# EthanD11/RS-VIO

Hardware: AMD Instinct MI355X
Metric: stereo frames/sec (tracker+BA) on 752×480 EuRoC stream; BA ms/iter at window=10 (higher is better)
Workload: dtype f32 (tracker) / f64 (BA)

## Files before the change

rs-vio_amd/csrc/pyramid.hip:

```cpp
#include "pyramid.hpp"

namespace rsvio {

namespace {

constexpr int TW = 64;
constexpr int TH = 8;
constexpr int STRIP_COLS = 320;
constexpr size_t LDS_CAP = 64 << 10;

__device__ __forceinline__ float triangle_kernel(float x) {
    float ax = fabsf(x);
    return ax < 1.0f ? 1.0f - ax : 0.0f;
}

__global__ void make_taps_kernel(TapTable tab, int n_entries) {
    int e = blockIdx.x * blockDim.x + threadIdx.x;
    if (e >= n_entries) return;
    int in_len = tab.ent_in_len[e];
    int out_len = tab.ent_out_len[e];
    int o = tab.ent_out_idx[e];
    float ratio = (float)in_len / (float)out_len;
    float sratio = ratio < 1.0f ? 1.0f : ratio;
    float support = 1.0f * sratio;
    float inputc = ((float)o + 0.5f) * ratio;
    long long left = (long long)floorf(inputc - support);
    if (left < 0) left = 0;
    if (left > (long long)in_len - 1) left = in_len - 1;
    long long right = (long long)ceilf(inputc + support);
    if (right < left + 1) right = left + 1;
    if (right > (long long)in_len) right = in_len;
    inputc = inputc - 0.5f;
    int cnt = (int)(right - left);
    float* w = tab.weights + (size_t)e * tab.max_taps;
    float sum = 0.0f;
    for (int k = 0; k < cnt; ++k) {
        float wv = triangle_kernel(((float)(left + k) - inputc) / sratio);
        w[k] = wv;
        sum += wv;
    }
    for (int k = 0; k < cnt; ++k) w[k] = w[k] / sum;
    tab.left[e] = (int)left;
    tab.count[e] = cnt;
}

__global__ __launch_bounds__(256) void pyramid_kernel(PyrLaunch L, PyrIO io) {
    extern __shared__ uint32_t smem[];
    const int img = blockIdx.y;
    {
        const int fb = (int)blockIdx.x - (L.copy_blocks + L.tile_start[L.levels]);
        if (fb >= 0) {
            if (img == 0 && fb < io.fast_cells) {
                const uint8_t* s0 = io.psrc ? io.psrc : io.src[0];
                fast_cell(s0, io.fg, fb, nullptr, nullptr, 0, io.fast_pt, io.fast_aff,
                          reinterpret_cast<uint8_t*>(smem));
            }
            return;
        }
    }
    const uint8_t* __restrict__ src = io.psrc ? io.psrc + (size_t)img * L.w * L.h : io.src[img];
    uint8_t* __restrict__ dst_base = io.psrc ? io.pdst + (size_t)img * L.pyr_bytes : io.dst[img];
    int b = blockIdx.x;
    const bool aligned = ((reinterpret_cast<uintptr_t>(src) | reinterpret_cast<uintptr_t>(dst_base)) & 15) == 0;
    if (b < L.copy_blocks) {
        const size_t tot = (size_t)L.w * L.h;
        if (!aligned) {
            for (size_t i = (size_t)b * blockDim.x + threadIdx.x; i < tot; i += (size_t)L.copy_blocks * blockDim.x)
                dst_base[i] = src[i];
            return;
        }
        const size_t n16 = tot / 16;
        const uint4* s4 = reinterpret_cast<const uint4*>(src);
        uint4* d4 = reinterpret_cast<uint4*>(dst_base);
        for (size_t i = (size_t)b * blockDim.x + threadIdx.x; i < n16; i += (size_t)L.copy_blocks * blockDim.x)
            d4[i] = s4[i];
        size_t tail0 = n16 * 16;
        if (b == 0)
            for (size_t i = tail0 + threadIdx.x; i < tot; i += blockDim.x) dst_base[i] = src[i];
        return;
    }
    b -= L.copy_blocks;
    int lev = 1;
    while (lev < L.levels - 1 && b >= L.tile_start[lev + 1]) ++lev;
    b -= L.tile_start[lev];
    const int nw = (int)level_w(L.w, lev), nh = (int)level_h(L.h, lev);
    const int tw = L.tile_w[lev], th = L.tile_h[lev];
    const int tiles_x = (nw + tw - 1) / tw;
    const int tx = b % tiles_x, ty = b / tiles_x;
    const int ox0 = tx * tw, ox1 = min(ox0 + tw, nw);
    const int oy0 = ty * th, oy1 = min(oy0 + th, nh);
    const int rows = oy1 - oy0, cols_out = ox1 - ox0;
    const int hx = L.hx_ent[lev], vy = L.vy_ent[lev];
    const TapTable& T = L.tab;
    const int xl = T.left[hx + ox0];
    const int xr = T.left[hx + ox1 - 1] + T.count[hx + ox1 - 1];
    const int yl = T.left[vy + oy0];
    const int yr = T.left[vy + oy1 - 1] + T.count[vy + oy1 - 1];
    const int ncols = xr - xl, nrows = yr - yl;
    const int xa = xl & ~3, xoff = xl - xa;
    const int pd = (xr - xa + 3) >> 2;
    const bool direct = (L.direct >> lev) & 1;
    uint8_t* strip = reinterpret_cast<uint8_t*>(smem);
    if (!direct) {
        if (aligned && (L.w & 3) == 0) {
            const uint32_t* s32 = reinterpret_cast<const uint32_t*>(src);
            const int wd = (int)(L.w >> 2);
            for (int idx = threadIdx.x; idx < nrows * pd; idx += blockDim.x) {
                const int r = idx / pd, d = idx - r * pd;
                smem[idx] = s32[(size_t)(yl + r) * wd + (xa >> 2) + d];
            }
        } else {
            for (int idx = threadIdx.x; idx < nrows * pd * 4; idx += blockDim.x) {
                const int r = idx / (pd * 4), c = idx - r * pd * 4;
                strip[idx] = (xa + c < (int)L.w) ? src[(size_t)(yl + r) * L.w + xa + c] : 0;
            }
        }
    }
    float* tmp = reinterpret_cast<float*>(smem + (direct ? 0 : nrows * pd));
    __syncthreads();
    for (int idx = threadIdx.x; idx < rows * ncols; idx += blockDim.x) {
        const int r = idx / ncols, c = idx - r * ncols;
        const int e = vy + oy0 + r;
        const int vl = T.left[e], vc = T.count[e];
        const float* __restrict__ vw = T.weights + (size_t)e * T.max_taps;
        float acc = 0.0f;
        if (!direct) {
            const uint8_t* col = strip + (vl - yl) * pd * 4 + xoff + c;
            for (int k = 0; k < vc; ++k) acc += (float)col[k * pd * 4] * vw[k];
        } else {
            const uint8_t* __restrict__ col = src + (size_t)vl * L.w + xl + c;
            for (int k = 0; k < vc; k += 8) {
                float px[8];
#pragma unroll
                for (int u = 0; u < 8; ++u) px[u] = (k + u < vc) ? (float)col[(size_t)(k + u) * L.w] : 0.0f;
#pragma unroll
                for (int u = 0; u < 8; ++u)
                    if (k + u < vc) acc += px[u] * vw[k + u];
            }
        }
        tmp[r * ncols + c] = acc;
    }
    __syncthreads();
    uint8_t* __restrict__ dst = dst_base + level_offset(L.w, L.h, lev);
    for (int idx = threadIdx.x; idx < rows * cols_out; idx += blockDim.x) {
        const int r = idx / cols_out, c = idx - r * cols_out;
        const int e = hx + ox0 + c;
        const int hl = T.left[e] - xl, hc = T.count[e];
        const float* __restrict__ hw = T.weights + (size_t)e * T.max_taps;
        const float* __restrict__ row = tmp + r * ncols + hl;
        float acc = 0.0f;
        for (int k = 0; k < hc; ++k) acc += row[k] * hw[k];
        float cl = acc < 0.0f ? 0.0f : (acc > 255.0f ? 255.0f : acc);
        dst[(size_t)(oy0 + r) * nw + ox0 + c] = (uint8_t)roundf(cl);
    }
}

}

void PyramidPlan::init(int w_, int h_, int levels_) {
    w = w_;
    h = h_;
    levels = levels_;
    if (levels < 1 || levels > kMaxLevels) throw std::invalid_argument("levels must be in [1, 8]");
    if (w < 16 || h < 16) throw std::invalid_argument("image too small");
    std::vector<int> in_len, out_len, out_idx;
    float max_ratio = 1.0f;
    memset(&launch, 0, sizeof(launch));
    for (int i = 1; i < levels; ++i) {
        int nw = (int)level_w(w, i), nh = (int)level_h(h, i);
        if (nw < 1 || nh < 1) throw std::invalid_argument("too many levels for image size");
        launch.hx_ent[i] = (int)in_len.size();
        for (int o = 0; o < nw; ++o) { in_len.push_back(w); out_len.push_back(nw); out_idx.push_back(o); }
        launch.vy_ent[i] = (int)in_len.size();
        for (int o = 0; o < nh; ++o) { in_len.push_back(h); out_len.push_back(nh); out_idx.push_back(o); }
        float rx = (float)w / nw, ry = (float)h / nh;
        max_ratio = std::max(max_ratio, std::max(rx, ry));
        launch.tile_h[i] = std::max(1, std::min(TH, (int)(16.0f / ry)));
        launch.tile_w[i] = std::max(1, std::min(TW, (int)std::floor((STRIP_COLS - 2.0f * rx - 4.0f) / rx)));
    }
    n_entries = (int)in_len.size();
    max_taps = (int)std::ceil(2.0f * max_ratio) + 4;
    int tiles = 0;
    for (int i = 1; i < levels; ++i) {
        launch.tile_start[i] = tiles;
        int nw = (int)level_w(w, i), nh = (int)level_h(h, i);
        tiles += ((nw + launch.tile_w[i] - 1) / launch.tile_w[i]) * ((nh + launch.tile_h[i] - 1) / launch.tile_h[i]);
    }
    launch.tile_start[levels] = tiles;
    launch.copy_blocks = std::max(1, (int)(((size_t)w * h / 16 + 255) / 256 / 4));
    total_blocks = launch.copy_blocks + tiles;
    launch.w = (uint32_t)w;
    launch.h = (uint32_t)h;
    launch.levels = levels;
    launch.pyr_bytes = level_offset(w, h, levels);
    if (n_entries > 0) {
        i_in.alloc(n_entries); i_out.alloc(n_entries); i_idx.alloc(n_entries);
        d_left.alloc(n_entries); d_count.alloc(n_entries);
        d_w.alloc((size_t)n_entries * max_taps);
        RSVIO_HIP(hipMemcpy(i_in.p, in_len.data(), sizeof(int) * n_entries, hipMemcpyHostToDevice));
        RSVIO_HIP(hipMemcpy(i_out.p, out_len.data(), sizeof(int) * n_entries, hipMemcpyHostToDevice));
        RSVIO_HIP(hipMemcpy(i_idx.p, out_idx.data(), sizeof(int) * n_entries, hipMemcpyHostToDevice));
        TapTable t;
        t.left = d_left.p; t.count = d_count.p; t.weights = d_w.p; t.max_taps = max_taps;
        t.ent_in_len = i_in.p; t.ent_out_len = i_out.p; t.ent_out_idx = i_idx.p;
        hipLaunchKernelGGL(make_taps_kernel, dim3((n_entries + 255) / 256), dim3(256), 0, 0, t, n_entries);
        RSVIO_HIP(hipGetLastError());
        RSVIO_HIP(hipDeviceSynchronize());
        launch.tab = t;
        std::vector<int> left(n_entries), count(n_entries);
        RSVIO_HIP(hipMemcpy(left.data(), d_left.p, sizeof(int) * n_entries, hipMemcpyDeviceToHost));
        RSVIO_HIP(hipMemcpy(count.data(), d_count.p, sizeof(int) * n_entries, hipMemcpyDeviceToHost));
        for (int i = 1; i < levels; ++i) {
            const int nw = (int)level_w(w, i), nh = (int)level_h(h, i);
            const int tw = launch.tile_w[i], th = launch.tile_h[i];
            size_t strip = 0, vert = 0;
            for (int ox0 = 0; ox0 < nw; ox0 += tw) {
                const int ox1 = std::min(ox0 + tw, nw);
                const int xl = left[launch.hx_ent[i] + ox0];
                const int xr = left[launch.hx_ent[i] + ox1 - 1] + count[launch.hx_ent[i] + ox1 - 1];
                const size_t pd = (size_t)(xr - (xl & ~3) + 3) / 4;
                for (int oy0 = 0; oy0 < nh; oy0 += th) {
                    const int oy1 = std::min(oy0 + th, nh);
                    const int yl = left[launch.vy_ent[i] + oy0];
                    const int yr = left[launch.vy_ent[i] + oy1 - 1] + count[launch.vy_ent[i] + oy1 - 1];
                    strip = std::max(strip, 4 * pd * (size_t)(yr - yl));
                    vert = std::max(vert, 4 * (size_t)(oy1 - oy0) * (size_t)(xr - xl));
                }
            }
            if (vert > LDS_CAP) throw std::invalid_argument("image too wide for the pyramid tile");
            if (strip + vert > LDS_CAP) launch.direct |= 1u << i;
            lds_bytes = std::max(lds_bytes, ((launch.direct >> i) & 1) ? vert : strip + vert);
        }
    }
}

void PyramidPlan::enqueue(const PyrIO& io, int n_img, hipStream_t s) const {
    if (n_img <= 0) return;
    if (n_img > (io.psrc ? 65535 : kMaxPyrIO)) throw std::invalid_argument("too many images per pyramid launch");
    const size_t lds = io.fast_cells > 0 ? std::max(lds_bytes, (size_t)io.fg.g * io.fg.g) : lds_bytes;
    hipLaunchKernelGGL(pyramid_kernel, dim3(total_blocks + std::max(io.fast_cells, 0), n_img), dim3(256), lds, s,
                       launch, io);
    RSVIO_HIP(hipGetLastError());
}

void PyramidPlan::enqueue(const uint8_t* d_imgs, int n_img, uint8_t* d_pyrs, hipStream_t s) const {
    for (int i0 = 0; i0 < n_img; i0 += 65535) {
        PyrIO io{};
        io.psrc = d_imgs + (size_t)i0 * w * h;
        io.pdst = d_pyrs + (size_t)i0 * pyr_bytes();
        enqueue(io, std::min(65535, n_img - i0), s);
    }
}

}
```

Before: 5175.

## Restructure pyramid kernel: wave-per-row staging, packed vertical pass, register horizontal taps

Strip loads in the pyramid downsampling kernel now go wave-by-row with several rows batched per thread for memory-level parallelism. The vertical pass reads packed 4-byte words from LDS and accumulates four columns at once. The horizontal pass keeps each lane's tap weights in registers and reuses them across the rows a wave handles. Tile height and the row budget grow so more rows share a block, and waves_per_eu is pinned at 8. The aims are fewer LDS and global transactions and less integer division, at the cost of more register pressure and of lanes sitting idle when a tile has fewer than 64 output columns.

After: 5121. 1.0% lower.

```diff
diff --git a/rs-vio_amd/csrc/pyramid.hip b/rs-vio_amd/csrc/pyramid.hip
--- a/rs-vio_amd/csrc/pyramid.hip
+++ b/rs-vio_amd/csrc/pyramid.hip
@@ -5,7 +5,10 @@
 namespace {
 
 constexpr int TW = 64;
-constexpr int TH = 8;
+constexpr int TH = 12;
+constexpr int ROW_BUDGET = 24;
+constexpr int kStage = 8;
+constexpr int kHReg = 16;
 constexpr int STRIP_COLS = 320;
 constexpr size_t LDS_CAP = 64 << 10;
 
@@ -44,7 +47,7 @@
     tab.count[e] = cnt;
 }
 
-__global__ __launch_bounds__(256) void pyramid_kernel(PyrLaunch L, PyrIO io) {
+__global__ __launch_bounds__(256) __attribute__((amdgpu_waves_per_eu(8, 8))) void pyramid_kernel(PyrLaunch L, PyrIO io) {
     extern __shared__ uint32_t smem[];
     const int img = blockIdx.y;
     {
@@ -92,23 +95,31 @@
     const int rows = oy1 - oy0, cols_out = ox1 - ox0;
     const int hx = L.hx_ent[lev], vy = L.vy_ent[lev];
     const TapTable& T = L.tab;
-    const int xl = T.left[hx + ox0];
-    const int xr = T.left[hx + ox1 - 1] + T.count[hx + ox1 - 1];
-    const int yl = T.left[vy + oy0];
-    const int yr = T.left[vy + oy1 - 1] + T.count[vy + oy1 - 1];
+    const int xl = T.left[hx + ox0], xe = T.left[hx + ox1 - 1], xc = T.count[hx + ox1 - 1];
+    const int yl = T.left[vy + oy0], ye = T.left[vy + oy1 - 1], yc = T.count[vy + oy1 - 1];
+    const int xr = xe + xc, yr = ye + yc;
     const int ncols = xr - xl, nrows = yr - yl;
+    const int wv = __builtin_amdgcn_readfirstlane((int)(threadIdx.x >> 6)), lane = threadIdx.x & 63;
     const int xa = xl & ~3, xoff = xl - xa;
     const int pd = (xr - xa + 3) >> 2;
     const bool direct = (L.direct >> lev) & 1;
     uint8_t* strip = reinterpret_cast<uint8_t*>(smem);
     if (!direct) {
         if (aligned && (L.w & 3) == 0) {
-            const uint32_t* s32 = reinterpret_cast<const uint32_t*>(src);
+            const uint32_t* s32 = reinterpret_cast<const uint32_t*>(src) + (xa >> 2);
             const int wd = (int)(L.w >> 2);
-            for (int idx = threadIdx.x; idx < nrows * pd; idx += blockDim.x) {
-                const int r = idx / pd, d = idx - r * pd;
-                smem[idx] = s32[(size_t)(yl + r) * wd + (xa >> 2) + d];
-            }
+            for (int r0 = wv; r0 < nrows; r0 += 4 * kStage)
+                for (int d = lane; d < pd; d += 64) {
+                    uint32_t v[kStage];
+#pragma unroll
+                    for (int u = 0; u < kStage; ++u) {
+                        const int r = min(r0 + 4 * u, nrows - 1);
+                        v[u] = s32[(size_t)(yl + r) * wd + d];
+                    }
+#pragma unroll
+                    for (int u = 0; u < kStage; ++u)
+                        if (r0 + 4 * u < nrows) smem[(r0 + 4 * u) * pd + d] = v[u];
+                }
         } else {
             for (int idx = threadIdx.x; idx < nrows * pd * 4; idx += blockDim.x) {
                 const int r = idx / (pd * 4), c = idx - r * pd * 4;
@@ -118,16 +129,45 @@
     }
     float* tmp = reinterpret_cast<float*>(smem + (direct ? 0 : nrows * pd));
     __syncthreads();
-    for (int idx = threadIdx.x; idx < rows * ncols; idx += blockDim.x) {
-        const int r = idx / ncols, c = idx - r * ncols;
-        const int e = vy + oy0 + r;
-        const int vl = T.left[e], vc = T.count[e];
-        const float* __restrict__ vw = T.weights + (size_t)e * T.max_taps;
-        float acc = 0.0f;
-        if (!direct) {
-            const uint8_t* col = strip + (vl - yl) * pd * 4 + xoff + c;
-            for (int k = 0; k < vc; ++k) acc += (float)col[k * pd * 4] * vw[k];
-        } else {
+    if (!direct) {
+        for (int r = wv; r < rows; r += 4) {
+            const int e = vy + oy0 + r;
+            const int vl = T.left[e], vc = T.count[e];
+            const float* __restrict__ vw = T.weights + (size_t)e * T.max_taps;
+            const uint32_t* srow = smem + (vl - yl) * pd;
+            float* __restrict__ out = tmp + r * ncols - xoff;
+            for (int d = lane; d < pd; d += 64) {
+                float a[4] = {0.0f, 0.0f, 0.0f, 0.0f};
+                for (int k0 = 0; k0 < vc; k0 += 4) {
+                    uint32_t px[4];
+                    float wk[4];
+#pragma unroll
+                    for (int u = 0; u < 4; ++u) {
+                        const int k = min(k0 + u, vc - 1);
+                        px[u] = srow[k * pd + d];
+                        wk[u] = vw[k];
+                    }
+#pragma unroll
+                    for (int u = 0; u < 4; ++u)
+                        if (k0 + u < vc) {
+#pragma unroll
+                            for (int j = 0; j < 4; ++j) a[j] += (float)((px[u] >> (8 * j)) & 255u) * wk[u];
+                        }
+                }
+#pragma unroll
+                for (int j = 0; j < 4; ++j) {
+                    const int c = 4 * d + j - xoff;
+                    if (c >= 0 && c < ncols) out[4 * d + j] = a[j];
+                }
+            }
+        }
+    } else {
+        for (int idx = threadIdx.x; idx < rows * ncols; idx += blockDim.x) {
+            const int r = idx / ncols, c = idx - r * ncols;
+            const int e = vy + oy0 + r;
+            const int vl = T.left[e], vc = T.count[e];
+            const float* __restrict__ vw = T.weights + (size_t)e * T.max_taps;
+            float acc = 0.0f;
             const uint8_t* __restrict__ col = src + (size_t)vl * L.w + xl + c;
             for (int k = 0; k < vc; k += 8) {
                 float px[8];
@@ -137,21 +177,45 @@
                 for (int u = 0; u < 8; ++u)
                     if (k + u < vc) acc += px[u] * vw[k + u];
             }
-        }
-        tmp[r * ncols + c] = acc;
+            tmp[r * ncols + c] = acc;
+        }
     }
     __syncthreads();
     uint8_t* __restrict__ dst = dst_base + level_offset(L.w, L.h, lev);
-    for (int idx = threadIdx.x; idx < rows * cols_out; idx += blockDim.x) {
-        const int r = idx / cols_out, c = idx - r * cols_out;
-        const int e = hx + ox0 + c;
-        const int hl = T.left[e] - xl, hc = T.count[e];
-        const float* __restrict__ hw = T.weights + (size_t)e * T.max_taps;
+    const bool on = lane < cols_out;
+    const int eh = hx + ox0 + (on ? lane : 0);
+    const int hl = T.left[eh] - xl, hc = on ? T.count[eh] : 0;
+    const float* __restrict__ hw = T.weights + (size_t)eh * T.max_taps;
+    const bool in_regs = __ballot(hc > kHReg) == 0;
+    const int klast = max(hc, 1) - 1;
+    float wr[kHReg];
+    if (in_regs) {
+#pragma unroll
+        for (int k0 = 0; k0 < kHReg; k0 += 4) {
+            if (__ballot(k0 < hc) == 0) break;
+#pragma unroll
+            for (int u = 0; u < 4; ++u) wr[k0 + u] = hw[min(k0 + u, klast)];
+        }
+    }
+    for (int r = wv; r < rows; r += 4) {
         const float* __restrict__ row = tmp + r * ncols + hl;
         float acc = 0.0f;
-        for (int k = 0; k < hc; ++k) acc += row[k] * hw[k];
+        if (in_regs) {
+#pragma unroll
+            for (int k0 = 0; k0 < kHReg; k0 += 4) {
+                if (__ballot(k0 < hc) == 0) break;
+                float v[4];
+#pragma unroll
+                for (int u = 0; u < 4; ++u) v[u] = row[min(k0 + u, klast)];
+#pragma unroll
+                for (int u = 0; u < 4; ++u)
+                    if (k0 + u < hc) acc += v[u] * wr[k0 + u];
+            }
+        } else {
+            for (int k = 0; k < hc; ++k) acc += row[k] * hw[k];
+        }
         float cl = acc < 0.0f ? 0.0f : (acc > 255.0f ? 255.0f : acc);
-        dst[(size_t)(oy0 + r) * nw + ox0 + c] = (uint8_t)roundf(cl);
+        if (on) dst[(size_t)(oy0 + r) * nw + ox0 + lane] = (uint8_t)roundf(cl);
     }
 }
 
@@ -175,7 +239,7 @@
         for (int o = 0; o < nh; ++o) { in_len.push_back(h); out_len.push_back(nh); out_idx.push_back(o); }
         float rx = (float)w / nw, ry = (float)h / nh;
         max_ratio = std::max(max_ratio, std::max(rx, ry));
-        launch.tile_h[i] = std::max(1, std::min(TH, (int)(16.0f / ry)));
+        launch.tile_h[i] = std::max(1, std::min(TH, (int)((float)ROW_BUDGET / ry)));
         launch.tile_w[i] = std::max(1, std::min(TW, (int)std::floor((STRIP_COLS - 2.0f * rx - 4.0f) / rx)));
     }
     n_entries = (int)in_len.size();
```
